# SwagMag1213/image-segmentation-project

Hardware: AMD Instinct MI355X
Metric: images/sec + mIoU, 512x512 U-Net bf16 at 1/2/4/8 MI355X (higher is better)
Workload: dtype bf16; 1 GPU; Base U-Net resnet34 no-attention train step (fwd+bce+bwd+Adam); global_batch=16, image=512x512, parallelism=dp1, fp8=False

## Files before the change

### image-segmentation-project_amd/csrc/conv_fl.hip

```cpp
#include <cstdio>

#include "common.h"
#include "kernels.h"

namespace unet {

void conv_kernel_tag(const char* tag);

namespace {

constexpr int kNC = 4, kNL = 4, kNW = kNC + kNL, kCOT = 64, kRW = 4, kFN = 4, kTH = 16;
constexpr int kHW = 18;
constexpr int kHPix = (kTH + 2) * kHW;
constexpr int kHIns = (kHPix + 7) / 8;
constexpr int kHBytes = kHIns * 1024;
constexpr int kWIns = 9 * kCOT / 16;
constexpr int kWBytes = kWIns * 1024;
constexpr int kOffH0 = 0, kOffW0 = kHBytes, kOffW1 = kOffW0 + kWBytes, kOffH1 = kOffW1 + kWBytes;
constexpr int kOffCst = kOffH1 + kHBytes;
constexpr int kNCst = 5;
constexpr int kLds = kOffCst + kNCst * kCOT * 4;
static_assert(kLds <= 163840, "LDS");
static_assert(256 * 256 <= kWBytes + kHBytes, "transpose buffer fits W1 | H1");
static_assert(kTH == kNC * kRW, "rows");
constexpr int kItems = 4;
constexpr int kWPer = kWIns / kNL;
constexpr int kHPer = (kHIns + kNL - 1) / kNL;
static_assert(kWIns % kNL == 0, "weight DMA per loader");

__device__ __forceinline__ int fl_off(int row, int chunk) { return row * 128 + ((chunk ^ (row & 6)) << 4); }
__device__ __forceinline__ int ws_off(int row, int chunk) { return row * 64 + ((chunk ^ ((row >> 1) & 2)) << 4); }
__device__ __forceinline__ int tp_off(int px, int c16) { return px * 256 + ((c16 ^ (px & 15)) << 4); }

__device__ __forceinline__ void wait_vm_h(int n) {
  if (n == 11) wait_vmcnt<11>();
  else wait_vmcnt<10>();
}
__device__ __forceinline__ void barrier_lds() {
  asm volatile("s_waitcnt lgkmcnt(0)" ::: "memory");
  __builtin_amdgcn_s_barrier();
  asm volatile("" ::: "memory");
}

}

constexpr int EP_FOLD = 1, EP_ADD = 2, EP_FBWD = 4, EP_STATS = 8, EP_RELU = 16, EP_RT = 32;

__device__ __forceinline__ void fl_ld8(const float* p, float (&d)[8]) {
  const f32x4 x0 = *reinterpret_cast<const f32x4*>(p), x1 = *reinterpret_cast<const f32x4*>(p + 4);
  d[0] = x0[0]; d[1] = x0[1]; d[2] = x0[2]; d[3] = x0[3]; d[4] = x1[0]; d[5] = x1[1]; d[6] = x1[2]; d[7] = x1[3];
}

template <bool FLIP, bool TWO>
__device__ __forceinline__ void fl_item(const ConvFwdArgs& a, const char* T, const float* cst, const float (&kb)[8],
                                        const float (&km)[8], const float (&mu)[8], const float (&is)[8], int q8, int px,
                                        int pix, int cob, bool fold, bool want_add, bool fbwd, bool stats,
                                        bool relu, const uint4& uadd, const uint4& uact, const uint4& uy,
                                        const uint4& uy2, float (&s0)[8], float (&s1)[8], float (&s2)[8]) {
  const f32x4 lo = *reinterpret_cast<const f32x4*>(T + tp_off(px, 2 * (q8 >> 3)));
  const f32x4 hi = *reinterpret_cast<const f32x4*>(T + tp_off(px, 2 * (q8 >> 3) + 1));
  float v[8] = {lo[0], lo[1], lo[2], lo[3], hi[0], hi[1], hi[2], hi[3]};
  float kb_[8];
  if (TWO) fl_ld8(cst + q8, kb_);
  if (fold) {
#pragma unroll
    for (int e = 0; e < 8; ++e) v[e] = v[e] * km[e] + kb[e];
  } else {
#pragma unroll
    for (int e = 0; e < 8; ++e) v[e] += TWO ? kb_[e] : kb[e];
  }
  if (want_add) {
    float ad[8];
    unpack8(uadd, ad);
#pragma unroll
    for (int e = 0; e < 8; ++e) v[e] += ad[e];
  }
  if (!FLIP && relu) {
#pragma unroll
    for (int e = 0; e < 8; ++e) v[e] = fmaxf(v[e], 0.f);
  }
  if (fbwd) {
    float m[8];
    unpack8(uact, m);
#pragma unroll
    for (int e = 0; e < 8; ++e)
      if (!(m[e] > 0.f)) v[e] = 0.f;
  }
  const uint4 ob = pack8(v);
  if (UNET_ABL != 4) *reinterpret_cast<uint4*>(a.y + (size_t)pix * a.ldy + cob * kCOT + q8) = ob;
  if (fbwd) {
    float dz[8], yv[8];
    unpack8(ob, dz);
    unpack8(uy, yv);
    float mu_[8], is_[8];
    if (TWO) {
      fl_ld8(cst + kCOT + q8, mu_);
      fl_ld8(cst + 2 * kCOT + q8, is_);
    }
#pragma unroll
    for (int e = 0; e < 8; ++e) {
      s0[e] += dz[e];
      s1[e] += dz[e] * (yv[e] - (TWO ? mu_[e] : mu[e])) * (TWO ? is_[e] : is[e]);
    }
    if constexpr (TWO) {
      float y2[8];
      unpack8(uy2, y2);
      const f32x4 n0 = *reinterpret_cast<const f32x4*>(cst + 3 * kCOT + q8);
      const f32x4 n1 = *reinterpret_cast<const f32x4*>(cst + 3 * kCOT + q8 + 4);
      const f32x4 j0 = *reinterpret_cast<const f32x4*>(cst + 4 * kCOT + q8);
      const f32x4 j1 = *reinterpret_cast<const f32x4*>(cst + 4 * kCOT + q8 + 4);
      const float mu2[8] = {n0[0], n0[1], n0[2], n0[3], n1[0], n1[1], n1[2], n1[3]};
      const float is2[8] = {j0[0], j0[1], j0[2], j0[3], j1[0], j1[1], j1[2], j1[3]};
#pragma unroll
      for (int e = 0; e < 8; ++e) s2[e] += dz[e] * (y2[e] - mu2[e]) * is2[e];
    }
  } else if (stats) {
#pragma unroll
    for (int e = 0; e < 8; ++e) { s0[e] += v[e]; s1[e] += v[e] * v[e]; }
  }
}

template <bool FLIP, bool TWO, int EP>
__global__ void __launch_bounds__(kNW * 64) conv3x3_fl_kernel(ConvFwdArgs a, int ncb, int nitems) {
  extern __shared__ __attribute__((aligned(16))) char smem[];
  float* cst = reinterpret_cast<float*>(smem + kOffCst);
  TSTAMP_RT(a.tim, 30);
  TSTAMP(a.tim, 0);
  const int tid = threadIdx.x, lane = tid & 63;
  const int wave = __builtin_amdgcn_readfirstlane(tid >> 6);
  const int slot = xcd_remap(blockIdx.x, gridDim.x);
  int item = slot;
  if (item >= nitems) return;
  const int tq = a.Q >> 4, tp = a.P / kTH;
  const int NSUB = a.C >> 5;
  constexpr bool RT = EP & EP_RT;
  const bool fbwd = RT ? FLIP && a.bb.sums != nullptr : (EP & EP_FBWD) != 0;
  const bool stats = RT ? a.stats != nullptr || fbwd : (EP & EP_STATS) != 0;
  const bool fold = RT ? !FLIP && a.fold_on : (EP & EP_FOLD) != 0;
  const bool want_add = RT ? a.add != nullptr : (EP & EP_ADD) != 0;
  const bool relu = RT ? a.fold_relu != 0 : (EP & EP_RELU) != 0;
  const int cob = item % ncb;

  if (wave < kNC) {
    const int aoff = ws_off(lane & 15, lane >> 4);
    int boff[kRW + 2][3];
#pragma unroll
    for (int h = 0; h < kRW + 2; ++h)
#pragma unroll
      for (int d = 0; d < 3; ++d) boff[h][d] = fl_off((wave * kRW + h) * kHW + d + (lane & 15), lane >> 4);
    TSTAMP(a.tim, 1);
    int stg = 0;
    for (;;) {
      f32x4 acc[kRW][kFN];
#pragma unroll
      for (int j = 0; j < kRW; ++j)
#pragma unroll
        for (int i = 0; i < kFN; ++i) acc[j][i] = f32x4{0.f, 0.f, 0.f, 0.f};
      for (int s = 0; s < NSUB; ++s, ++stg) {
        barrier_lds();
        if (stg < 16) TSTAMP(a.tim, 2 + stg);
        const char* W = smem + ((s & 1) ? kOffW1 : kOffW0);
        const char* H = smem + (((s >> 1) & 1) ? kOffH1 : kOffH0);
        const int pb = (s & 1) << 6;
        if (UNET_ABL == 1) continue;
#pragma unroll
        for (int r = 0; r < 3; ++r)
#pragma unroll
          for (int c = 0; c < 3; ++c) {
            bf16x8 A[kFN];
#pragma unroll
            for (int i = 0; i < kFN; ++i)
              A[i] = *reinterpret_cast<const bf16x8*>(W + ((r * 3 + c) * kCOT + i * 16) * 64 + aoff);
            const int dr = FLIP ? 2 - r : r, dc = FLIP ? 2 - c : c;
#pragma unroll
            for (int j = 0; j < kRW; ++j) {
              const bf16x8 B = *reinterpret_cast<const bf16x8*>(H + (boff[j + dr][dc] ^ pb));
#pragma unroll
              for (int i = 0; i < kFN; ++i)
                acc[j][i] = __builtin_amdgcn_mfma_f32_16x16x32_bf16(A[i], B, acc[j][i], 0, 0, 0);
            }
          }
      }
      TSTAMP(a.tim, 20);
      barrier_lds();
      char* T = smem + kOffW1;
#pragma unroll
      for (int j = 0; j < kRW; ++j)
#pragma unroll
        for (int i = 0; i < kFN; ++i) {
          const int px = (wave * kRW + j) * 16 + (lane & 15);
          *reinterpret_cast<f32x4*>(T + tp_off(px, i * 4 + (lane >> 4))) = acc[j][i];
        }
      item += gridDim.x;
      if (item >= nitems) break;
    }
    barrier_lds();
    if (stats) {
      __builtin_amdgcn_s_barrier();
      __builtin_amdgcn_s_barrier();
    }
    return;
  }

  const int lw = wave - kNC, lt = tid - kNC * 64;
  const int nh = (kHIns - lw + kNL - 1) / kNL;
  const i32x4 xr = make_rsrc_sgpr(a.x, (unsigned)((size_t)a.N * a.H * a.W * a.ldx * 2));
  const i32x4 wr = make_rsrc_sgpr(a.wch, (unsigned)((size_t)a.C * 9 * a.Cout * 2));
  unsigned woff[kWPer], hoff[kHPer];
#pragma unroll
  for (int k = 0; k < kWPer; ++k) {
    const int ins = lw + k * kNL;
    const int tap = ins >> 2, co = (ins & 3) * 16 + (lane >> 2);
    const int lch = (lane & 3) ^ ((co >> 1) & 2);
    woff[k] = (unsigned)(((tap * a.Cout + cob * kCOT + co) * 32 + lch * 8) * 2);
  }
  auto set_hoff = [&](int it) {
    const int t = it / ncb;
    const int n = t / (tp * tq), rem = t - n * (tp * tq);
    const int oh0 = (rem / tq) * kTH, ow0 = (rem % tq) << 4;
#pragma unroll
    for (int k = 0; k < kHPer; ++k) {
      const int hp = (lw + k * kNL) * 8 + (lane >> 3);
      const int hr = hp / kHW, hc = hp - hr * kHW;
      const int ih = oh0 - 1 + hr, iw = ow0 - 1 + hc;
      const int q = (lane & 7) ^ (hp & 6);
      hoff[k] = kOOB;
      if (hp < kHPix && (unsigned)ih < (unsigned)a.H && (unsigned)iw < (unsigned)a.W)
        hoff[k] = (unsigned)((((n * a.H + ih) * a.W + iw) * a.ldx + q * 8) * 2);
    }
  };
  auto issue_w = [&](int t, int b) {
    char* dst = smem + (b ? kOffW1 : kOffW0);
    const unsigned so = (unsigned)t * 9u * (unsigned)a.Cout * 64u;
#pragma unroll
    for (int k = 0; k < kWPer; ++k) glds16_asm(wr, dst + (lw + k * kNL) * 1024, woff[k], so);
  };
  auto issue_h = [&](int sc, int b) {
    char* dst = smem + (b ? kOffH1 : kOffH0);
    const unsigned so = (unsigned)sc * 128u;
#pragma unroll
    for (int k = 0; k < kHPer; ++k)
      if (k < nh) glds16_asm(xr, dst + (lw + k * kNL) * 1024, hoff[k], so);
  };
  [[maybe_unused]] constexpr int LT = kNC * 64;
  set_hoff(item);
  TSTAMP_TH(a.tim, 23, LT);
  issue_w(0, 0);
  issue_h(0, 0);
  TSTAMP_TH(a.tim, 24, LT);
  static_assert(kCOT == 64, "loader wave 0 = loader threads 0..kCOT-1");
  if (lw == 0) {
    const int c = lt, co = cob * kCOT + c;
    float b = a.bias ? a.bias[co] : 0.f, c1 = 0.f, c2 = 0.f, c3 = 0.f, c4 = 0.f;
    if (fold) {
      float sc, sh, m, is, var;
      bn_scale_shift(a.fold, co, sc, sh, m, is, var);
      b = b * sc + sh;
      c1 = sc;
    } else if (fbwd) {
      c1 = a.bb.mean[co];
      c2 = a.bb.invstd[co];
      if (TWO) { c3 = a.bb.mean2[co]; c4 = a.bb.invstd2[co]; }
    }
    cst[c] = b; cst[kCOT + c] = c1; cst[2 * kCOT + c] = c2; cst[3 * kCOT + c] = c3; cst[4 * kCOT + c] = c4;
  }
  const int q8 = (lane & 7) * 8;
  auto px_of = [&](int k) {
    const int j = (lane >> 3) + 8 * k;
    return 16 * (j >> 2) + 4 * lw + (j & 3);
  };
  float s0[8], s1[8], s2[8];
#pragma unroll
  for (int e = 0; e < 8; ++e) s0[e] = s1[e] = s2[e] = 0.f;
  constexpr int NI = 2 * kItems;
  constexpr int NP = TWO ? 0 : NI;
  int ep_pix0 = 0;
  auto pix_of = [&](int k) {
    const int px = px_of(k);
    return ep_pix0 + (px >> 4) * a.Q + (px & 15);
  };
  auto load_ops = [&](int k, uint4& oa, uint4& om, uint4& oy, uint4& oy2) {
    const size_t pp = (size_t)pix_of(k);
    const int co = cob * kCOT + q8;
    oa = want_add ? *reinterpret_cast<const uint4*>(a.add + pp * a.ldadd + co) : make_uint4(0, 0, 0, 0);
    om = fbwd ? *reinterpret_cast<const uint4*>(a.bb.act + pp * a.bb.ldact + co) : make_uint4(0, 0, 0, 0);
    oy = fbwd ? *reinterpret_cast<const uint4*>(a.bb.y + pp * a.bb.ldy + co) : make_uint4(0, 0, 0, 0);
    if constexpr (TWO) oy2 = fbwd ? *reinterpret_cast<const uint4*>(a.bb.y2 + pp * a.bb.ldy2 + co) : make_uint4(0, 0, 0, 0);
    else oy2 = make_uint4(0, 0, 0, 0);
  };
  constexpr int NPA = NP > 0 ? NP : 1;
  uint4 opa[NPA], opm[NPA], opy[NPA], opy2[TWO ? NPA : 1];
  auto epilogue = [&]() {
    float kb[8], km[8], mu[8], is[8];
#pragma unroll
    for (int e = 0; e < 8; ++e) kb[e] = km[e] = mu[e] = is[e] = 0.f;
    if (!TWO) fl_ld8(cst + q8, kb);
    if (fold) fl_ld8(cst + kCOT + q8, km);
    if (fbwd && !TWO) {
      fl_ld8(cst + kCOT + q8, mu);
      fl_ld8(cst + 2 * kCOT + q8, is);
    }
    if constexpr (NP > 0) {
#pragma unroll
      for (int k = 0; k < NI; ++k) {
        fl_item<FLIP, TWO>(a, smem + kOffW1, cst, kb, km, mu, is, q8, px_of(k), pix_of(k), cob, fold, want_add, fbwd,
                           stats, relu, opa[k], opm[k], opy[k], opy2[TWO ? k : 0], s0, s1, s2);
        asm volatile("" ::: "memory");
      }
    } else {
      constexpr int G = 4;
#pragma unroll
      for (int k0 = 0; k0 < NI; k0 += G) {
        uint4 la[G], lm[G], ly[G], ly2[G];
#pragma unroll
        for (int k = 0; k < G; ++k) load_ops(k0 + k, la[k], lm[k], ly[k], ly2[k]);
#pragma unroll
        for (int k = 0; k < G; ++k) {
          fl_item<FLIP, TWO>(a, smem + kOffW1, cst, kb, km, mu, is, q8, px_of(k0 + k), pix_of(k0 + k), cob, fold,
                             want_add, fbwd, stats, relu, la[k], lm[k], ly[k], ly2[k], s0, s1, s2);
          asm volatile("" ::: "memory");
        }
      }
    }
    asm volatile("s_waitcnt lgkmcnt(0)" ::: "memory");
  };
  constexpr int NOPS = (RT || NP == NI) ? -1 : NP * (((EP & EP_ADD) ? 1 : 0) + ((EP & EP_FBWD) ? (TWO ? 3 : 2) : 0));
  auto fetch_operands = [&]() {
#pragma unroll
    for (int k = 0; k < NP; ++k) load_ops(k, opa[k], opm[k], opy[k], opy2[TWO ? k : 0]);
  };
  (void)opa; (void)opm; (void)opy; (void)opy2;
  bool pending = false;
  int nit = 0;
  for (;;) {
    const int next = item + gridDim.x;
    if constexpr (NOPS > 0) {
      if (pending) wait_vmcnt<(NOPS > 0 ? NOPS : 0)>();
      else wait_vmcnt<0>();
    } else {
      wait_vmcnt<0>();
    }
    if (nit == 0) TSTAMP_TH(a.tim, 25, LT);
    if (nit == 1) TSTAMP_TH(a.tim, 27, LT);
    __builtin_amdgcn_s_barrier();
    if (pending) epilogue();
    if (UNET_ABL != 2) {
      issue_w(1, 1);
      if (2 < NSUB) issue_h(1, 1);
    }
    for (int s = 1; s < NSUB - 1; ++s) {
      if (s & 1) wait_vm_h(nh);
      else wait_vmcnt<0>();
      __builtin_amdgcn_s_barrier();
      if (UNET_ABL != 2) {
        issue_w(s + 1, (s + 1) & 1);
        if (!(s & 1) && s + 2 < NSUB) issue_h((s >> 1) + 1, ((s >> 1) + 1) & 1);
      }
    }
    wait_vmcnt<0>();
    __builtin_amdgcn_s_barrier();
    {
      const int t = item / ncb;
      const int n = t / (tp * tq), rem = t - n * (tp * tq);
      const int oh0 = (rem / tq) * kTH, ow0 = (rem % tq) << 4;
      ep_pix0 = (n * a.P + oh0) * a.Q + ow0;
    }
    if constexpr (NOPS < 0) fetch_operands();
    if (nit == 0) TSTAMP_TH(a.tim, 26, LT);
    ++nit;
    if (next < nitems) {
      set_hoff(next);
      issue_w(0, 0);
      issue_h(0, 0);
    }
    if constexpr (NOPS >= 0) fetch_operands();
    __builtin_amdgcn_s_barrier();
    pending = true;
    item = next;
    if (item >= nitems) break;
  }
  asm volatile("s_waitcnt lgkmcnt(0)" ::: "memory");
  __builtin_amdgcn_s_barrier();
  TSTAMP_TH(a.tim, 28, LT);
  epilogue();
  TSTAMP_TH(a.tim, 21, LT);
  if (!stats) {
    TSTAMP_RT_TH(a.tim, 31, LT);
    return;
  }
  float* red = reinterpret_cast<float*>(smem + kOffH0);
  {
    const int sl = lt >> 3;
#pragma unroll
    for (int e = 0; e < 8; ++e) {
      red[(sl * kCOT + q8 + e) * 3 + 0] = s0[e];
      red[(sl * kCOT + q8 + e) * 3 + 1] = s1[e];
      red[(sl * kCOT + q8 + e) * 3 + 2] = s2[e];
    }
  }
  barrier_lds();
  if (lt < (TWO ? 3 : 2) * kCOT) {
    const int c = lt % kCOT, which = lt / kCOT;
    float p[4] = {0.f, 0.f, 0.f, 0.f};
#pragma unroll
    for (int sl = 0; sl < 32; ++sl) p[sl & 3] += red[(sl * kCOT + c) * 3 + which];
    const float tsum = (p[0] + p[1]) + (p[2] + p[3]);
    const int co = cob * kCOT + c;
    const size_t rep = (size_t)(blockIdx.x % kStatRep) * 2 * a.Cout;
    if (which == 2) atomicAdd(a.bb.sums2 + rep + a.Cout + co, (double)tsum);
    else atomicAdd((fbwd ? a.bb.sums : a.stats) + rep + which * a.Cout + co, (double)tsum);
  }
  __builtin_amdgcn_s_barrier();
  TSTAMP_TH(a.tim, 22, LT);
  TSTAMP_RT_TH(a.tim, 31, LT);
}

static int cu_count() { return device_cu_count(); }

bool conv3x3_fl_geom(int C, int Cout, int P, int Q) {
  return C > 0 && Cout > 0 && P > 0 && Q > 0 && C % 128 == 0 && Cout % kCOT == 0 && P % kTH == 0 && Q % 16 == 0;
}

bool conv3x3_fl_shape(int N, int C, int Cout, int P, int Q) {
  if (!conv3x3_fl_geom(C, Cout, P, Q)) return false;
  return (long long)N * (P / kTH) * (Q / 16) * (Cout / kCOT) >= cu_count();
}

hipError_t launch_conv3x3_fl(const ConvFwdArgs& a, int mode, hipStream_t st) {
  const bool flip = mode == 1;
  if (!a.wch || a.R != 3 || a.S != 3 || a.stride != 1 || a.pad != 1 || a.x2 || a.ysplit || a.xform)
    return hipErrorInvalidValue;
  if (a.N <= 0 || a.H != a.P || a.W != a.Q || !conv3x3_fl_geom(a.C, a.Cout, a.P, a.Q)) return hipErrorInvalidValue;
  if (a.ldx % 8 || a.ldy % 8 || (a.add && a.ldadd % 8)) return hipErrorInvalidValue;
  if (flip && (a.fold_on || a.stats || (a.bb.sums && (a.bb.ldact % 8 || a.bb.ldy % 8 ||
                                                     (a.bb.y2 && a.bb.ldy2 % 8)))))
    return hipErrorInvalidValue;
  if (!flip && a.bb.sums) return hipErrorInvalidValue;
  if ((size_t)a.N * a.H * a.W * a.ldx * 2 >= 0x80000000ull || (size_t)a.C * 9 * a.Cout * 2 >= 0x80000000ull ||
      (size_t)a.N * a.P * a.Q >= 0x80000000ull)
    return hipErrorInvalidValue;
  const int ncb = a.Cout / kCOT;
  const int nitems = a.N * (a.P / kTH) * (a.Q / 16) * ncb;
  int grid = cu_count() / ncb * ncb;
  if (a.grid_cap > 0 && a.grid_cap < grid) grid = a.grid_cap / ncb * ncb;
  if (grid < ncb) grid = ncb;
  if (grid > nitems) grid = nitems;
  const bool two = flip && a.bb.sums && a.bb.y2;
  const bool fbwd = flip && a.bb.sums;
  const int ep = (!flip && a.fold_on ? EP_FOLD : 0) | (a.add ? EP_ADD : 0) | (fbwd ? EP_FBWD : 0) |
                 (a.stats || fbwd ? EP_STATS : 0) | (!flip && a.fold_relu ? EP_RELU : 0);
  int sel = EP_RT;
  if (!flip && (ep == EP_STATS || ep == 0)) sel = ep;
  if (flip && !two && (ep == 0 || ep == EP_ADD || ep == (EP_FBWD | EP_STATS) || ep == (EP_FBWD | EP_STATS | EP_ADD)))
    sel = ep;
  char tag[96];
  std::snprintf(tag, sizeof(tag), "conv3x3_fl_kernel<%s, %s, %d>", flip ? "true" : "false", two ? "true" : "false",
                sel);
  conv_kernel_tag(tag);
  const dim3 g(grid), b(kNW * 64);
#define FL_LAUNCH(F, T, E) hipLaunchKernelGGL((conv3x3_fl_kernel<F, T, E>), g, b, kLds, st, a, ncb, nitems)
  if (!flip) {
    if (sel == EP_STATS) FL_LAUNCH(false, false, EP_STATS);
    else if (sel == 0) FL_LAUNCH(false, false, 0);
    else FL_LAUNCH(false, false, EP_RT);
  } else if (two) {
    FL_LAUNCH(true, true, EP_RT);
  } else {
    if (sel == (EP_FBWD | EP_STATS)) FL_LAUNCH(true, false, EP_FBWD | EP_STATS);
    else if (sel == (EP_FBWD | EP_STATS | EP_ADD)) FL_LAUNCH(true, false, EP_FBWD | EP_STATS | EP_ADD);
    else if (sel == EP_ADD) FL_LAUNCH(true, false, EP_ADD);
    else if (sel == 0) FL_LAUNCH(true, false, 0);
    else FL_LAUNCH(true, false, EP_RT);
  }
#undef FL_LAUNCH
  return hipGetLastError();
}


constexpr int kW2Bytes = 9 * kCOT * 128;
constexpr int k2OffH0 = kW2Bytes, k2OffH1 = k2OffH0 + kHBytes, k2OffCst = k2OffH1 + kHBytes;
constexpr int k2OffXss = k2OffCst + 3 * kCOT * 4;
constexpr int k2Lds = k2OffXss + 2 * 64 * 4;
constexpr int EP_XF = 64;
static_assert(k2Lds <= 163840, "LDS");
static_assert(256 * 128 <= kHBytes, "bf16 tile fits a halo buffer");
__device__ __forceinline__ int t2_off(int px, int c16) { return px * 128 + ((c16 ^ (px & 7)) << 4); }

template <bool FBWD, int Q0, int Q1, bool TV = false>
__device__ __forceinline__ void ws2_items(const ConvFwdArgs& a, const char* T, int cob, int pix0, int sw, int lane,
                                          const float (&mu)[8], const float (&is)[8], float (&s0)[8],
                                          float (&s1)[8], const uint4* tv = nullptr) {
  const int c8 = (lane & 7) * 8;
  uint4 om[Q1 - Q0], oy[Q1 - Q0];
  if constexpr (FBWD) {
#pragma unroll
    for (int q = Q0; q < Q1; ++q) {
      const int px = (sw + 4 * q) * 8 + (lane >> 3);
      const size_t gp = (size_t)(pix0 + (px >> 4) * a.Q + (px & 15));
      om[q - Q0] = *reinterpret_cast<const uint4*>(a.bb.act + gp * a.bb.ldact + cob * kCOT + c8);
      oy[q - Q0] = *reinterpret_cast<const uint4*>(a.bb.y + gp * a.bb.ldy + cob * kCOT + c8);
    }
  }
#pragma unroll
  for (int q = Q0; q < Q1; ++q) {
    const int px = (sw + 4 * q) * 8 + (lane >> 3);
    const size_t gp = (size_t)(pix0 + (px >> 4) * a.Q + (px & 15));
    uint4 o = TV ? tv[q - Q0] : *reinterpret_cast<const uint4*>(T + t2_off(px, lane & 7));
    if constexpr (FBWD) {
      float v[8], m[8], yv[8];
      unpack8(o, v);
      unpack8(om[q - Q0], m);
      unpack8(oy[q - Q0], yv);
#pragma unroll
      for (int e = 0; e < 8; ++e) {
        if (!(m[e] > 0.f)) v[e] = 0.f;
        s0[e] += v[e];
        s1[e] += v[e] * (yv[e] - mu[e]) * is[e];
      }
      o = pack8(v);
    }
    if (UNET_ABL != 4) *reinterpret_cast<uint4*>(a.y + gp * a.ldy + cob * kCOT + c8) = o;
  }
}

template <bool FLIP, int EP>
__global__ void __launch_bounds__(kNW * 64) conv3x3_ws2_kernel(ConvFwdArgs a, int ncb, int nitems) {
  extern __shared__ __attribute__((aligned(16))) char smem[];
  float* cst = reinterpret_cast<float*>(smem + k2OffCst);
  TSTAMP_RT(a.tim, 30);
  TSTAMP(a.tim, 0);
  const int tid = threadIdx.x, lane = tid & 63;
  const int wave = __builtin_amdgcn_readfirstlane(tid >> 6);
  const int slot = xcd_remap(blockIdx.x, gridDim.x);
  if (slot >= nitems) return;
  const size_t rep = (size_t)(blockIdx.x % kStatRep) * 2 * a.Cout;
  const int cob = slot % ncb;
  const int tq = a.Q >> 4, tp = a.P / kTH;
  constexpr bool FBWD = FLIP && (EP & EP_FBWD), ADD = (EP & EP_ADD) != 0, STATS = (EP & EP_STATS) != 0;
  constexpr bool XF = !FLIP && (EP & EP_XF);
  float* xss = reinterpret_cast<float*>(smem + k2OffXss);
  auto tile_pix0 = [&](int it) {
    const int t = it / ncb;
    const int n = t / (tp * tq), rem = t - n * (tp * tq);
    return (n * a.P + (rem / tq) * kTH) * a.Q + ((rem % tq) << 4);
  };
  const char* Wl = smem;

  if (wave < kNC) {
    const int aoff = fl_off(lane & 15, lane >> 4), g = lane >> 4;
    int boff[kRW + 2][3];
#pragma unroll
    for (int h = 0; h < kRW + 2; ++h)
#pragma unroll
      for (int d = 0; d < 3; ++d) boff[h][d] = fl_off((wave * kRW + h) * kHW + d + (lane & 15), lane >> 4);
    float q0[kFN][4], q1[kFN][4];
#pragma unroll
    for (int i = 0; i < kFN; ++i)
#pragma unroll
      for (int e = 0; e < 4; ++e) q0[i][e] = q1[i][e] = 0.f;
    if constexpr (XF) {
      if (blockIdx.x == 0) bn_finalize(a.xbn, 0, a.xbn.C);
      __builtin_amdgcn_s_barrier();
    }
    TSTAMP(a.tim, 1);
    int b = 0, k = 0;
    for (int it = slot; it < nitems; it += gridDim.x, b ^= 1, ++k) {
      const int pix0 = tile_pix0(it);
      __builtin_amdgcn_s_barrier();
      asm volatile("" ::: "memory");
      if (k < 8) TSTAMP(a.tim, 2 + 2 * k);
      uint2 uadd[kRW][kFN];
      if constexpr (ADD) {
#pragma unroll
        for (int j = 0; j < kRW; ++j) {
          const int px = (wave * kRW + j) * 16 + (lane & 15);
          const size_t gp = (size_t)(pix0 + (px >> 4) * a.Q + (px & 15));
#pragma unroll
          for (int i = 0; i < kFN; ++i)
            uadd[j][i] = *reinterpret_cast<const uint2*>(a.add + gp * a.ldadd + cob * kCOT + i * 16 + 4 * g);
        }
        asm volatile("" ::: "memory");
      }
      const char* H = smem + k2OffH0 + b * kHBytes;
      f32x4 acc[kRW][kFN];
#pragma unroll
      for (int j = 0; j < kRW; ++j)
#pragma unroll
        for (int i = 0; i < kFN; ++i) acc[j][i] = f32x4{0.f, 0.f, 0.f, 0.f};
      if (UNET_ABL != 1) {
#pragma unroll
        for (int p = 0; p < 2; ++p)
#pragma unroll
          for (int r = 0; r < 3; ++r)
#pragma unroll
            for (int c = 0; c < 3; ++c) {
              bf16x8 A[kFN];
#pragma unroll
              for (int i = 0; i < kFN; ++i)
                A[i] = *reinterpret_cast<const bf16x8*>(Wl + (r * 3 + c) * kCOT * 128 + i * 2048 + (aoff ^ (p << 6)));
              const int dr = FLIP ? 2 - r : r, dc = FLIP ? 2 - c : c;
#pragma unroll
              for (int j = 0; j < kRW; ++j) {
                const bf16x8 B = *reinterpret_cast<const bf16x8*>(H + (boff[j + dr][dc] ^ (p << 6)));
#pragma unroll
                for (int i = 0; i < kFN; ++i)
                  acc[j][i] = __builtin_amdgcn_mfma_f32_16x16x32_bf16(A[i], B, acc[j][i], 0, 0, 0);
              }
            }
      }
      if (k < 8) TSTAMP(a.tim, 3 + 2 * k);
      barrier_lds();
      char* T = smem + k2OffH0 + b * kHBytes;
#pragma unroll
      for (int i = 0; i < kFN; ++i) {
        float kb[4];
#pragma unroll
        for (int e = 0; e < 4; ++e) kb[e] = cst[i * 16 + 4 * g + e];
#pragma unroll
        for (int j = 0; j < kRW; ++j) {
          float v[4];
#pragma unroll
          for (int e = 0; e < 4; ++e) v[e] = acc[j][i][e] + kb[e];
          if constexpr (ADD) {
            const float ad[4] = {__uint_as_float(uadd[j][i].x << 16), __uint_as_float(uadd[j][i].x & 0xffff0000u),
                                 __uint_as_float(uadd[j][i].y << 16), __uint_as_float(uadd[j][i].y & 0xffff0000u)};
#pragma unroll
            for (int e = 0; e < 4; ++e) v[e] += ad[e];
          }
          if constexpr (!FLIP && STATS) {
#pragma unroll
            for (int e = 0; e < 4; ++e) { q0[i][e] += v[e]; q1[i][e] += v[e] * v[e]; }
          }
          const int px = (wave * kRW + j) * 16 + (lane & 15);
          *reinterpret_cast<uint2*>(T + t2_off(px, 2 * i + (g >> 1)) + (g & 1) * 8) =
              make_uint2(pack_bf2(v[0], v[1]), pack_bf2(v[2], v[3]));
        }
      }
      barrier_lds();
    }
    TSTAMP(a.tim, 20);
    float es0[8], es1[8], emu[8], eis[8];
#pragma unroll
    for (int e = 0; e < 8; ++e) es0[e] = es1[e] = 0.f;
    {
      const int ce8 = (lane & 7) * 8;
      if constexpr (FBWD) {
        fl_ld8(cst + kCOT + ce8, emu);
        fl_ld8(cst + 2 * kCOT + ce8, eis);
      }
      int lit = slot;
      while (lit + (int)gridDim.x < nitems) lit += gridDim.x;
      ws2_items<FBWD, 4, 8>(a, smem + k2OffH0 + (b ^ 1) * kHBytes, cob, tile_pix0(lit), wave, lane, emu, eis, es0,
                            es1);
    }
    if constexpr (FBWD) {
      float* red = reinterpret_cast<float*>(smem + k2OffH0 + b * kHBytes);
      const int sl = 32 + (tid >> 3), ce8 = (lane & 7) * 8;
#pragma unroll
      for (int e = 0; e < 8; ++e) {
        red[(sl * kCOT + ce8 + e) * 2 + 0] = es0[e];
        red[(sl * kCOT + ce8 + e) * 2 + 1] = es1[e];
      }
    }
    if constexpr (!FLIP && STATS) {
      float* red = reinterpret_cast<float*>(smem + k2OffH0 + b * kHBytes);
#pragma unroll
      for (int i = 0; i < kFN; ++i)
#pragma unroll
        for (int e = 0; e < 4; ++e) {
          red[(wave * 64 + lane) * 32 + i * 4 + e] = q0[i][e];
          red[(wave * 64 + lane) * 32 + 16 + i * 4 + e] = q1[i][e];
        }
    }
    __builtin_amdgcn_s_barrier();
    __builtin_amdgcn_s_barrier();
    return;
  }

  const int lw = wave - kNC, lt = tid - kNC * 64;
  const int nh = (kHIns - lw + kNL - 1) / kNL;
  const i32x4 xr = make_rsrc_sgpr(a.x, (unsigned)((size_t)a.N * a.H * a.W * a.ldx * 2));
  const i32x4 wr = make_rsrc_sgpr(a.w, (unsigned)((size_t)a.Cout * 9 * a.C * 2));
  [[maybe_unused]] constexpr int LT = kNC * 64;
  unsigned hoff[kHPer];
  auto set_hoff = [&](int it) {
    const int t = it / ncb;
    const int n = t / (tp * tq), rem = t - n * (tp * tq);
    const int oh0 = (rem / tq) * kTH, ow0 = (rem % tq) << 4;
#pragma unroll
    for (int k = 0; k < kHPer; ++k) {
      const int hp = (lw + k * kNL) * 8 + (lane >> 3);
      const int hr = hp / kHW, hc = hp - hr * kHW;
      const int ih = oh0 - 1 + hr, iw = ow0 - 1 + hc;
      const int q = (lane & 7) ^ (hp & 6);
      hoff[k] = kOOB;
      if (hp < kHPix && (unsigned)ih < (unsigned)a.H && (unsigned)iw < (unsigned)a.W)
        hoff[k] = (unsigned)((((n * a.H + ih) * a.W + iw) * a.ldx + q * 8) * 2);
    }
  };
  const unsigned l0 = lds_addr(smem);
  auto issue_h = [&](int bb) {
    const unsigned dst = l0 + k2OffH0 + bb * kHBytes;
#pragma unroll
    for (int k = 0; k < kHPer; ++k)
      if (k < nh) glds16_asm_at(xr, dst + (lw + k * kNL) * 1024, hoff[k], 0u);
  };
  if constexpr (XF) {
    if (lt < 64) {
      float m, iv, var;
      bn_scale_shift(a.xbn, lt, xss[lt], xss[64 + lt], m, iv, var);
    }
  }
  TSTAMP_TH(a.tim, 23, LT);
  for (int ins = lw; ins < 9 * kCOT / 8; ins += kNL) {
    const int row = ins * 8 + (lane >> 3);
    const int co = row % kCOT, tap = row / kCOT;
    const int q = (lane & 7) ^ (row & 6);
    const unsigned off = (unsigned)((((cob * kCOT + co) * 9 + tap) * a.C + q * 8) * 2);
    glds16_asm_at(wr, l0 + ins * 1024, off, 0u);
  }
  int item = slot;
  set_hoff(item);
  issue_h(0);
  TSTAMP_TH(a.tim, 24, LT);
  if (lt < kCOT) {
    const int co = cob * kCOT + lt;
    cst[lt] = a.bias ? a.bias[co] : 0.f;
    cst[kCOT + lt] = FBWD ? a.bb.mean[co] : 0.f;
    cst[2 * kCOT + lt] = FBWD ? a.bb.invstd[co] : 0.f;
  }
  if constexpr (XF) __builtin_amdgcn_s_barrier();
  auto xform_halo = [&](int bb, int it) {
    char* Hb = smem + k2OffH0 + bb * kHBytes;
    const int t = it / ncb;
    const int n = t / (tp * tq), rem = t - n * (tp * tq);
    const int oh0 = (rem / tq) * kTH, ow0 = (rem % tq) << 4;
#pragma unroll
    for (int k = 0; k < kHPer; ++k) {
      if (k >= nh || hoff[k] == kOOB) continue;
      const int hp = (lw + k * kNL) * 8 + (lane >> 3);
      const int c0 = ((lane & 7) ^ (hp & 6)) * 8;
      uint4* q = reinterpret_cast<uint4*>(Hb + (lw + k * kNL) * 1024 + lane * 16);
      float v[8];
      unpack8(*q, v);
#pragma unroll
      for (int e = 0; e < 8; ++e) v[e] = v[e] * xss[c0 + e] + xss[64 + c0 + e];
#pragma unroll
      for (int e = 0; e < 8; ++e) v[e] = v[e] > 0.f ? v[e] : 0.f;
      const uint4 o = pack8(v);
      *q = o;
      const int hr = hp / kHW, hc = hp - hr * kHW;
      if (cob == 0 && hr >= 1 && hr <= kTH && hc >= 1 && hc <= 16 && UNET_ABL != 4)
        *reinterpret_cast<uint4*>(a.xh + ((size_t)(n * a.H + oh0 - 1 + hr) * a.W + ow0 - 1 + hc) * a.ldxh + c0) = o;
    }
  };
  const int c8 = (lane & 7) * 8;
  float s0[8], s1[8], mu[8], is[8];
#pragma unroll
  for (int e = 0; e < 8; ++e) s0[e] = s1[e] = 0.f;
  bool have_cst = false;
  uint4 tv[8];
  auto epi_read = [&](int tb) {
    const char* T = smem + k2OffH0 + tb * kHBytes;
#pragma unroll
    for (int q = 0; q < 8; ++q) tv[q] = *reinterpret_cast<const uint4*>(T + t2_off((lw + 4 * q) * 8 + (lane >> 3), lane & 7));
    asm volatile("s_waitcnt lgkmcnt(0)" ::: "memory");
  };
  auto epilogue = [&](int tb, int pix0) {
    if (FBWD && !have_cst) {
      fl_ld8(cst + kCOT + c8, mu);
      fl_ld8(cst + 2 * kCOT + c8, is);
      have_cst = true;
    }
    ws2_items<FBWD, 0, 8, true>(a, nullptr, cob, pix0, lw, lane, mu, is, s0, s1, tv);
  };
  int k = 0, b = 0, prev_pix0 = 0;
  for (; item < nitems; item += gridDim.x, b ^= 1, ++k) {
    const int next = item + gridDim.x;
    if (!XF || k == 0) wait_vmcnt<0>();
    if (XF && k == 0) xform_halo(b, item);
    if (k == 0) TSTAMP_TH(a.tim, 25, LT);
    if (k == 1) TSTAMP_TH(a.tim, 27, LT);
    __builtin_amdgcn_s_barrier();
    if (k > 0) epi_read(b ^ 1);
    if (k == 0) TSTAMP_TH(a.tim, 26, LT);
    if (next < nitems) {
      set_hoff(next);
      issue_h(b ^ 1);
    }
    if (k > 0) epilogue(b ^ 1, prev_pix0);
    prev_pix0 = tile_pix0(item);
    if (XF && next < nitems) {
      wait_vmcnt<0>();
      xform_halo(b ^ 1, next);
    }
    __builtin_amdgcn_s_barrier();
    __builtin_amdgcn_s_barrier();
  }
  {
    if (FBWD && !have_cst) {
      fl_ld8(cst + kCOT + c8, mu);
      fl_ld8(cst + 2 * kCOT + c8, is);
    }
    ws2_items<FBWD, 0, 4>(a, smem + k2OffH0 + (b ^ 1) * kHBytes, cob, prev_pix0, lw, lane, mu, is, s0, s1);
  }
  TSTAMP_TH(a.tim, 21, LT);
  float* red = reinterpret_cast<float*>(smem + k2OffH0 + b * kHBytes);
  if constexpr (FBWD) {
    const int sl = lt >> 3;
#pragma unroll
    for (int e = 0; e < 8; ++e) {
      red[(sl * kCOT + c8 + e) * 2 + 0] = s0[e];
      red[(sl * kCOT + c8 + e) * 2 + 1] = s1[e];
    }
  }
  __builtin_amdgcn_s_barrier();
  if constexpr (!FLIP && STATS) {
    if (lt < 2 * kCOT) {
      const int co = lt % kCOT, which = lt / kCOT;
      const int i = co >> 4, gg = (co >> 2) & 3, e = co & 3;
      float p[4] = {0.f, 0.f, 0.f, 0.f};
#pragma unroll
      for (int w = 0; w < kNC; ++w)
#pragma unroll
        for (int l = 0; l < 16; ++l) p[l & 3] += red[(w * 64 + gg * 16 + l) * 32 + which * 16 + i * 4 + e];
      const float tsum = (p[0] + p[1]) + (p[2] + p[3]);
      atomicAdd(a.stats + rep + which * a.Cout + cob * kCOT + co, (double)tsum);
    }
  }
  if constexpr (FBWD) {
    if (lt < 2 * kCOT) {
      const int c = lt % kCOT, which = lt / kCOT;
      float p[4] = {0.f, 0.f, 0.f, 0.f};
#pragma unroll
      for (int sl = 0; sl < 64; ++sl) p[sl & 3] += red[(sl * kCOT + c) * 2 + which];
      const float tsum = (p[0] + p[1]) + (p[2] + p[3]);
      atomicAdd(a.bb.sums + rep + which * a.Cout + cob * kCOT + c, (double)tsum);
    }
  }
  __builtin_amdgcn_s_barrier();
  TSTAMP_TH(a.tim, 22, LT);
  TSTAMP_RT_TH(a.tim, 31, LT);
}

bool conv3x3_ws2_ok(const ConvFwdArgs& a, bool flip) {
  if (a.C != 64 || a.Cout % kCOT || a.P % kTH || a.Q % 16 || a.H != a.P || a.W != a.Q) return false;
  if (a.R != 3 || a.S != 3 || a.stride != 1 || a.pad != 1 || a.x2 || a.ysplit || a.fold_on) return false;
  if (a.xform && (flip || !a.xh || a.ldxh % 8)) return false;
  if (a.ldx % 8 || a.ldy % 8 || (a.add && a.ldadd % 4)) return false;
  if (!flip && (a.add || a.bb.sums)) return false;
  if (flip && (a.stats || (a.bb.sums && (a.bb.y2 || a.bb.ldact % 8 || a.bb.ldy % 8)))) return false;
  if ((size_t)a.N * a.H * a.W * a.ldx * 2 >= 0x80000000ull || (size_t)a.N * a.P * a.Q >= 0x80000000ull) return false;
  return true;
}

hipError_t launch_conv3x3_ws2(const ConvFwdArgs& a, int mode, hipStream_t st) {
  const bool flip = mode == 1;
  if (!conv3x3_ws2_ok(a, flip)) return hipErrorInvalidValue;
  const int ncb = a.Cout / kCOT;
  const int nitems = a.N * (a.P / kTH) * (a.Q / 16) * ncb;
  int grid = cu_count() / ncb * ncb;
  if (a.grid_cap > 0 && a.grid_cap < grid) grid = a.grid_cap / ncb * ncb;
  if (grid < ncb) grid = ncb;
  if (grid > nitems) grid = nitems;
  const bool fbwd = flip && a.bb.sums;
  const int ep = (a.add ? EP_ADD : 0) | (fbwd ? EP_FBWD : 0) | (a.stats || fbwd ? EP_STATS : 0) |
                 (!flip && a.xform ? EP_XF : 0);
  char tag[96];
  std::snprintf(tag, sizeof(tag), "conv3x3_ws2_kernel<%s, %d>", flip ? "true" : "false", ep);
  conv_kernel_tag(tag);
  const dim3 g(grid), bl(kNW * 64);
#define WS2_LAUNCH(F, E) hipLaunchKernelGGL((conv3x3_ws2_kernel<F, E>), g, bl, k2Lds, st, a, ncb, nitems)
  if (!flip) {
    if (ep == (EP_STATS | EP_XF)) WS2_LAUNCH(false, EP_STATS | EP_XF);
    else if (ep == EP_XF) WS2_LAUNCH(false, EP_XF);
    else if (ep == EP_STATS) WS2_LAUNCH(false, EP_STATS);
    else WS2_LAUNCH(false, 0);
  } else {
    switch (ep) {
      case EP_FBWD | EP_STATS: WS2_LAUNCH(true, EP_FBWD | EP_STATS); break;
      case EP_FBWD | EP_STATS | EP_ADD: WS2_LAUNCH(true, EP_FBWD | EP_STATS | EP_ADD); break;
      case EP_ADD: WS2_LAUNCH(true, EP_ADD); break;
      default: WS2_LAUNCH(true, 0); break;
    }
  }
#undef WS2_LAUNCH
  return hipGetLastError();
}

}
```

Baseline: 3100 images/sec.

## Split conv epilogue into LDS read and math phases overlapped with next-tile loads

The persistent conv3x3 kernel's epilogue is split into an LDS-read phase and a math phase. The math now runs after the next subtile's weight and halo loads have been issued, so it overlaps with memory traffic. The halo prefetch for the next item moves into the last sub-step, and operand prefetch now covers the TWO (dual-BN backward) path too, with per-channel constants hoisted out of the per-pixel loop. In exchange it holds more registers (all transposed values and operands live across the loop), which risks lower occupancy or spills, and it adds scheduling barriers.

```diff
diff --git a/image-segmentation-project_amd/csrc/conv_fl.hip b/image-segmentation-project_amd/csrc/conv_fl.hip
--- a/image-segmentation-project_amd/csrc/conv_fl.hip
+++ b/image-segmentation-project_amd/csrc/conv_fl.hip
@@ -1,4 +1,5 @@
 #include <cstdio>
+#include <type_traits>
 
 #include "common.h"
 #include "kernels.h"
@@ -52,22 +53,19 @@
 }
 
 template <bool FLIP, bool TWO>
-__device__ __forceinline__ void fl_item(const ConvFwdArgs& a, const char* T, const float* cst, const float (&kb)[8],
-                                        const float (&km)[8], const float (&mu)[8], const float (&is)[8], int q8, int px,
-                                        int pix, int cob, bool fold, bool want_add, bool fbwd, bool stats,
-                                        bool relu, const uint4& uadd, const uint4& uact, const uint4& uy,
-                                        const uint4& uy2, float (&s0)[8], float (&s1)[8], float (&s2)[8]) {
-  const f32x4 lo = *reinterpret_cast<const f32x4*>(T + tp_off(px, 2 * (q8 >> 3)));
-  const f32x4 hi = *reinterpret_cast<const f32x4*>(T + tp_off(px, 2 * (q8 >> 3) + 1));
+__device__ __forceinline__ void fl_item(const ConvFwdArgs& a, const f32x4& lo, const f32x4& hi, const float (&kb)[8],
+                                        const float (&km)[8], const float (&mu)[8], const float (&is)[8],
+                                        const float (&mu2)[8], const float (&is2)[8], size_t yo,
+                                        bool fold, bool want_add, bool fbwd, bool stats, bool relu, const uint4& uadd,
+                                        const uint4& uact, const uint4& uy, const uint4& uy2, float (&s0)[8],
+                                        float (&s1)[8], float (&s2)[8]) {
   float v[8] = {lo[0], lo[1], lo[2], lo[3], hi[0], hi[1], hi[2], hi[3]};
-  float kb_[8];
-  if (TWO) fl_ld8(cst + q8, kb_);
   if (fold) {
 #pragma unroll
     for (int e = 0; e < 8; ++e) v[e] = v[e] * km[e] + kb[e];
   } else {
 #pragma unroll
-    for (int e = 0; e < 8; ++e) v[e] += TWO ? kb_[e] : kb[e];
+    for (int e = 0; e < 8; ++e) v[e] += kb[e];
   }
   if (want_add) {
     float ad[8];
@@ -87,32 +85,25 @@
       if (!(m[e] > 0.f)) v[e] = 0.f;
   }
   const uint4 ob = pack8(v);
-  if (UNET_ABL != 4) *reinterpret_cast<uint4*>(a.y + (size_t)pix * a.ldy + cob * kCOT + q8) = ob;
+  if (UNET_ABL != 4) *reinterpret_cast<uint4*>(a.y + yo) = ob;
   if (fbwd) {
     float dz[8], yv[8];
     unpack8(ob, dz);
     unpack8(uy, yv);
-    float mu_[8], is_[8];
-    if (TWO) {
-      fl_ld8(cst + kCOT + q8, mu_);
-      fl_ld8(cst + 2 * kCOT + q8, is_);
-    }
 #pragma unroll
     for (int e = 0; e < 8; ++e) {
       s0[e] += dz[e];
-      s1[e] += dz[e] * (yv[e] - (TWO ? mu_[e] : mu[e])) * (TWO ? is_[e] : is[e]);
+      if constexpr (TWO) s1[e] = __builtin_fmaf(dz[e] * (yv[e] - mu[e]), is[e], s1[e]);
+      else s1[e] += dz[e] * (yv[e] - mu[e]) * is[e];
     }
     if constexpr (TWO) {
       float y2[8];
       unpack8(uy2, y2);
-      const f32x4 n0 = *reinterpret_cast<const f32x4*>(cst + 3 * kCOT + q8);
-      const f32x4 n1 = *reinterpret_cast<const f32x4*>(cst + 3 * kCOT + q8 + 4);
-      const f32x4 j0 = *reinterpret_cast<const f32x4*>(cst + 4 * kCOT + q8);
-      const f32x4 j1 = *reinterpret_cast<const f32x4*>(cst + 4 * kCOT + q8 + 4);
-      const float mu2[8] = {n0[0], n0[1], n0[2], n0[3], n1[0], n1[1], n1[2], n1[3]};
-      const float is2[8] = {j0[0], j0[1], j0[2], j0[3], j1[0], j1[1], j1[2], j1[3]};
-#pragma unroll
-      for (int e = 0; e < 8; ++e) s2[e] += dz[e] * (y2[e] - mu2[e]) * is2[e];
+#pragma unroll
+      for (int e = 0; e < 7; ++e) s2[e] = __builtin_fmaf(dz[e] * (y2[e] - mu2[e]), is2[e], s2[e]);
+      float t7 = dz[7] * (y2[7] - mu2[7]) * is2[7];
+      asm volatile("" : "+v"(t7));
+      s2[7] += t7;
     }
   } else if (stats) {
 #pragma unroll
@@ -218,12 +209,14 @@
     const int t = it / ncb;
     const int n = t / (tp * tq), rem = t - n * (tp * tq);
     const int oh0 = (rem / tq) * kTH, ow0 = (rem % tq) << 4;
+    int hl = lane;
+    asm volatile("" : "+v"(hl));
 #pragma unroll
     for (int k = 0; k < kHPer; ++k) {
-      const int hp = (lw + k * kNL) * 8 + (lane >> 3);
+      const int hp = (lw + k * kNL) * 8 + (hl >> 3);
       const int hr = hp / kHW, hc = hp - hr * kHW;
       const int ih = oh0 - 1 + hr, iw = ow0 - 1 + hc;
-      const int q = (lane & 7) ^ (hp & 6);
+      const int q = (hl & 7) ^ (hp & 6);
       hoff[k] = kOOB;
       if (hp < kHPix && (unsigned)ih < (unsigned)a.H && (unsigned)iw < (unsigned)a.W)
         hoff[k] = (unsigned)((((n * a.H + ih) * a.W + iw) * a.ldx + q * 8) * 2);
@@ -264,16 +257,17 @@
     }
     cst[c] = b; cst[kCOT + c] = c1; cst[2 * kCOT + c] = c2; cst[3 * kCOT + c] = c3; cst[4 * kCOT + c] = c4;
   }
+  int el = lane;
   const int q8 = (lane & 7) * 8;
   auto px_of = [&](int k) {
-    const int j = (lane >> 3) + 8 * k;
+    const int j = (el >> 3) + 8 * k;
     return 16 * (j >> 2) + 4 * lw + (j & 3);
   };
   float s0[8], s1[8], s2[8];
 #pragma unroll
   for (int e = 0; e < 8; ++e) s0[e] = s1[e] = s2[e] = 0.f;
   constexpr int NI = 2 * kItems;
-  constexpr int NP = TWO ? 0 : NI;
+  constexpr bool PF = !(FLIP && (RT || (EP & EP_FBWD)));
   int ep_pix0 = 0;
   auto pix_of = [&](int k) {
     const int px = px_of(k);
@@ -281,34 +275,63 @@
   };
   auto load_ops = [&](int k, uint4& oa, uint4& om, uint4& oy, uint4& oy2) {
     const size_t pp = (size_t)pix_of(k);
-    const int co = cob * kCOT + q8;
+    const int co = cob * kCOT + (el & 7) * 8;
     oa = want_add ? *reinterpret_cast<const uint4*>(a.add + pp * a.ldadd + co) : make_uint4(0, 0, 0, 0);
     om = fbwd ? *reinterpret_cast<const uint4*>(a.bb.act + pp * a.bb.ldact + co) : make_uint4(0, 0, 0, 0);
     oy = fbwd ? *reinterpret_cast<const uint4*>(a.bb.y + pp * a.bb.ldy + co) : make_uint4(0, 0, 0, 0);
     if constexpr (TWO) oy2 = fbwd ? *reinterpret_cast<const uint4*>(a.bb.y2 + pp * a.bb.ldy2 + co) : make_uint4(0, 0, 0, 0);
     else oy2 = make_uint4(0, 0, 0, 0);
   };
-  constexpr int NPA = NP > 0 ? NP : 1;
-  uint4 opa[NPA], opm[NPA], opy[NPA], opy2[TWO ? NPA : 1];
-  auto epilogue = [&]() {
-    float kb[8], km[8], mu[8], is[8];
-#pragma unroll
-    for (int e = 0; e < 8; ++e) kb[e] = km[e] = mu[e] = is[e] = 0.f;
-    if (!TWO) fl_ld8(cst + q8, kb);
+  uint4 opa[NI], opm[NI], opy[NI], opy2[TWO ? NI : 1];
+  f32x4 tv[NI][2];
+  auto epi_read = [&]() {
+    const char* T = smem + kOffW1;
+    asm volatile("" : "+v"(el));
+#pragma unroll
+    for (int k = 0; k < NI; ++k) {
+      tv[k][0] = *reinterpret_cast<const f32x4*>(T + tp_off(px_of(k), 2 * (el & 7)));
+      tv[k][1] = *reinterpret_cast<const f32x4*>(T + tp_off(px_of(k), 2 * (el & 7) + 1));
+    }
+    asm volatile("s_waitcnt lgkmcnt(0)" ::: "memory");
+  };
+  constexpr bool PRE = !TWO;
+  int toff[PRE ? NI : 1];
+  size_t yoff[PRE ? NI : 1];
+  auto y_off = [&](int k) { return (size_t)pix_of(k) * a.ldy + cob * kCOT + (el & 7) * 8; };
+  auto epi_math = [&](auto have, auto inl) {
+    constexpr bool HAVE = decltype(have)::value, INL = decltype(inl)::value;
+    static_assert(HAVE || !INL, "the tail form has its operands");
+    float kb[8], km[8], mu[8], is[8], mu2[8], is2[8];
+#pragma unroll
+    for (int e = 0; e < 8; ++e) kb[e] = km[e] = mu[e] = is[e] = mu2[e] = is2[e] = 0.f;
+    if constexpr (!INL || !PRE) asm volatile("" : "+v"(el));
+    const int q8 = (el & 7) * 8;
+    fl_ld8(cst + q8, kb);
     if (fold) fl_ld8(cst + kCOT + q8, km);
-    if (fbwd && !TWO) {
+    if (fbwd) {
       fl_ld8(cst + kCOT + q8, mu);
       fl_ld8(cst + 2 * kCOT + q8, is);
-    }
-    if constexpr (NP > 0) {
+      if constexpr (TWO) {
+        fl_ld8(cst + 3 * kCOT + q8, mu2);
+        fl_ld8(cst + 4 * kCOT + q8, is2);
+      }
+    }
+    if constexpr (HAVE) {
+      const char* T = smem + kOffW1;
 #pragma unroll
       for (int k = 0; k < NI; ++k) {
-        fl_item<FLIP, TWO>(a, smem + kOffW1, cst, kb, km, mu, is, q8, px_of(k), pix_of(k), cob, fold, want_add, fbwd,
-                           stats, relu, opa[k], opm[k], opy[k], opy2[TWO ? k : 0], s0, s1, s2);
+        f32x4 lo = tv[k][0], hi = tv[k][1];
+        if constexpr (INL) {
+          const int to = PRE ? toff[PRE ? k : 0] : tp_off(px_of(k), 2 * (el & 7));
+          lo = *reinterpret_cast<const f32x4*>(T + to);
+          hi = *reinterpret_cast<const f32x4*>(T + (to ^ 16));
+        }
+        fl_item<FLIP, TWO>(a, lo, hi, kb, km, mu, is, mu2, is2, INL && PRE ? yoff[PRE ? k : 0] : y_off(k), fold,
+                           want_add, fbwd, stats, relu, opa[k], opm[k], opy[k], opy2[TWO ? k : 0], s0, s1, s2);
         asm volatile("" ::: "memory");
       }
     } else {
-      constexpr int G = 4;
+      constexpr int G = TWO ? 2 : 4;
 #pragma unroll
       for (int k0 = 0; k0 < NI; k0 += G) {
         uint4 la[G], lm[G], ly[G], ly2[G];
@@ -316,38 +339,33 @@
         for (int k = 0; k < G; ++k) load_ops(k0 + k, la[k], lm[k], ly[k], ly2[k]);
 #pragma unroll
         for (int k = 0; k < G; ++k) {
-          fl_item<FLIP, TWO>(a, smem + kOffW1, cst, kb, km, mu, is, q8, px_of(k0 + k), pix_of(k0 + k), cob, fold,
-                             want_add, fbwd, stats, relu, la[k], lm[k], ly[k], ly2[k], s0, s1, s2);
+          fl_item<FLIP, TWO>(a, tv[k0 + k][0], tv[k0 + k][1], kb, km, mu, is, mu2, is2, y_off(k0 + k), fold, want_add,
+                             fbwd, stats, relu, la[k], lm[k], ly[k], ly2[k], s0, s1, s2);
           asm volatile("" ::: "memory");
         }
       }
     }
-    asm volatile("s_waitcnt lgkmcnt(0)" ::: "memory");
-  };
-  constexpr int NOPS = (RT || NP == NI) ? -1 : NP * (((EP & EP_ADD) ? 1 : 0) + ((EP & EP_FBWD) ? (TWO ? 3 : 2) : 0));
+  };
   auto fetch_operands = [&]() {
 #pragma unroll
-    for (int k = 0; k < NP; ++k) load_ops(k, opa[k], opm[k], opy[k], opy2[TWO ? k : 0]);
-  };
-  (void)opa; (void)opm; (void)opy; (void)opy2;
+    for (int k = 0; k < NI; ++k) load_ops(k, opa[k], opm[k], opy[k], opy2[TWO ? k : 0]);
+  };
+  constexpr std::true_type yes{};
+  constexpr std::false_type no{};
   bool pending = false;
   int nit = 0;
   for (;;) {
     const int next = item + gridDim.x;
-    if constexpr (NOPS > 0) {
-      if (pending) wait_vmcnt<(NOPS > 0 ? NOPS : 0)>();
-      else wait_vmcnt<0>();
-    } else {
-      wait_vmcnt<0>();
-    }
+    wait_vmcnt<0>();
     if (nit == 0) TSTAMP_TH(a.tim, 25, LT);
     if (nit == 1) TSTAMP_TH(a.tim, 27, LT);
     __builtin_amdgcn_s_barrier();
-    if (pending) epilogue();
+    if (pending) epi_read();
     if (UNET_ABL != 2) {
       issue_w(1, 1);
       if (2 < NSUB) issue_h(1, 1);
     }
+    if (pending) epi_math(std::bool_constant<PF>{}, no);
     for (int s = 1; s < NSUB - 1; ++s) {
       if (s & 1) wait_vm_h(nh);
       else wait_vmcnt<0>();
@@ -356,8 +374,13 @@
         issue_w(s + 1, (s + 1) & 1);
         if (!(s & 1) && s + 2 < NSUB) issue_h((s >> 1) + 1, ((s >> 1) + 1) & 1);
       }
-    }
-    wait_vmcnt<0>();
+      if (s == NSUB - 2 && next < nitems) {
+        set_hoff(next);
+        issue_h(0, 0);
+      }
+    }
+    if (next < nitems) wait_vm_h(nh);
+    else wait_vmcnt<0>();
     __builtin_amdgcn_s_barrier();
     {
       const int t = item / ncb;
@@ -365,24 +388,29 @@
       const int oh0 = (rem / tq) * kTH, ow0 = (rem % tq) << 4;
       ep_pix0 = (n * a.P + oh0) * a.Q + ow0;
     }
-    if constexpr (NOPS < 0) fetch_operands();
     if (nit == 0) TSTAMP_TH(a.tim, 26, LT);
     ++nit;
-    if (next < nitems) {
-      set_hoff(next);
-      issue_w(0, 0);
-      issue_h(0, 0);
-    }
-    if constexpr (NOPS >= 0) fetch_operands();
+    if (next >= nitems) break;
+    if constexpr (PF) fetch_operands();
+    issue_w(0, 0);
     __builtin_amdgcn_s_barrier();
     pending = true;
     item = next;
-    if (item >= nitems) break;
-  }
+  }
+  asm volatile("" : "+v"(el));
+  fetch_operands();
+  if constexpr (PRE) {
+#pragma unroll
+    for (int k = 0; k < NI; ++k) {
+      toff[k] = tp_off(px_of(k), 2 * (el & 7));
+      yoff[k] = y_off(k);
+    }
+  }
+  __builtin_amdgcn_s_barrier();
   asm volatile("s_waitcnt lgkmcnt(0)" ::: "memory");
   __builtin_amdgcn_s_barrier();
   TSTAMP_TH(a.tim, 28, LT);
-  epilogue();
+  epi_math(yes, yes);
   TSTAMP_TH(a.tim, 21, LT);
   if (!stats) {
     TSTAMP_RT_TH(a.tim, 31, LT);
```

After: 3126 images/sec, median of 6. No clear change (+0.8%).
